# huj31415/nbody3d-webgpu

Measured on AMD Instinct MI355X. Metric: pair-interactions/s, higher is better.
Workload: dtype f32; 1 GPU; N=262144 Plummer sphere, dt=1e-3, G=1, eps2=1e-4, i-sharded over 1 GPU(s); n=262144, kernel_variant=f32pk_symw_ipl16_j1_w2048_r32t128, parallelism=1gpu

## Files before the change

### include/nbody3d_hip.h

```cpp
#ifndef NBODY3D_HIP_H
#define NBODY3D_HIP_H

#include <stddef.h>
#include <stdint.h>

#ifdef __cplusplus
extern "C" {
#endif
#if defined(__GNUC__)
#pragma GCC visibility push(default)
#endif

#define NB_ABI_VERSION 2u
#define NB_ABI_MINOR 4u

typedef struct nb_sim nb_sim;

typedef enum nb_status {
    NB_OK = 0,
    NB_ERR_INVALID = 1,
    NB_ERR_NO_DEVICE = 2,
    NB_ERR_HIP = 3,
    NB_ERR_STATE = 4,
    NB_ERR_NOMEM = 5,
    NB_ERR_COMM = 6,
    NB_NOT_READY = 7
} nb_status;

typedef enum nb_precision { NB_F32 = 0, NB_F64 = 1 } nb_precision;

#define NB_FLAG_EXT_STREAM 1u
#define NB_FLAG_LDS_ONLY 4u
#define NB_FLAG_NO_FUSE 8u
#define NB_FLAG_POISON 16u

#define NB_FLAG_JPK_FENCED 32u

#define NB_FLAG_NO_SYM 64u

#define NB_FLAG_SYM_SHARD 128u

#define NB_FLAG_WHOLE_SWEEPS 256u

#define NB_FLAG_SINGLE_SWEEPS 512u

typedef enum nb_array { NB_BODIES = 0, NB_VEL = 1, NB_ACCEL = 2, NB_JERK = 3  } nb_array;

typedef enum nb_integrator { NB_INT_LEAPFROG = 0, NB_INT_HERMITE4 = 1 } nb_integrator;

typedef struct nb_config {
    uint32_t struct_size;
    uint32_t n;
    uint32_t precision;
    uint32_t tile;
    double eps2;
    int32_t device;
    uint32_t shard_begin;
    uint32_t shard_count;
    void *ext_stream;
    void *ext_bodies;
    uint32_t force_variant;
    uint32_t jsplit;
    uint32_t flags;
    uint32_t layer_budget_mib;
    uint32_t integrator;
    uint32_t reserved[3];
} nb_config;

uint32_t nb_abi_version(void);
uint32_t nb_abi_minor(void);

int nb_device_count(void);

int nb_create(const nb_config *cfg, nb_sim **out);

void nb_destroy(nb_sim *s);

// ... 108 lines not shown
```

### nbody3d-webgpu_amd/csrc/kernels/symmetric.hip.h

```cpp
#pragma once

namespace nb {

template <typename T> struct SymRowT { T x, y, z; };
using SymRow = SymRowT<float>;

constexpr uint32_t kFlushSteps = 4096;

template <int NG>
__device__ __forceinline__ void flush_resident_sums(float (*hi)[64], const int lane, const bool flushed, nb_f2 (&ax)[NG], nb_f2 (&ay)[NG], nb_f2 (&az)[NG])
{
    if (flushed) {
#pragma unroll
        for (int c = 0; c < NG; ++c) {
            hi[6 * c + 0][lane] += ax[c].x; hi[6 * c + 1][lane] += ay[c].x; hi[6 * c + 2][lane] += az[c].x;
            hi[6 * c + 3][lane] += ax[c].y; hi[6 * c + 4][lane] += ay[c].y; hi[6 * c + 5][lane] += az[c].y;
        }
    } else {
#pragma unroll
        for (int c = 0; c < NG; ++c) {
            hi[6 * c + 0][lane] = ax[c].x; hi[6 * c + 1][lane] = ay[c].x; hi[6 * c + 2][lane] = az[c].x;
            hi[6 * c + 3][lane] = ax[c].y; hi[6 * c + 4][lane] = ay[c].y; hi[6 * c + 5][lane] = az[c].y;
        }
    }
// ... 147 lines not shown
#pragma unroll
    for (int c = 0; c < NG; ++c) {
        out[(2 * c) * 64] = SymRow{ax[c].x, ay[c].x, az[c].x};
        out[(2 * c + 1) * 64] = SymRow{ax[c].y, ay[c].y, az[c].y};
    }
}

struct SymWK { uint32_t np, nsb, W, total_hi, total_lo, n_hi, zc, ups, r_layer0, t_layer0; };
#define SYMW_PLAN_PARAMS const uint32_t W_, const uint32_t ups_, const uint32_t nsb_, const uint32_t zc_, const uint32_t r_layer0_, const uint32_t t_layer0_
typedef uint32_t nb_u4 __attribute__((ext_vector_type(4)));
template <int TAIL>
__device__ __forceinline__ void symw_record_and_tail(const uint32_t* rec_at, nb_u4& rec, uint32_t (&tail)[TAIL])
{
    static_assert(TAIL == 1 || TAIL == 4, "f32: eps2; f64: G, eps2");
    constexpr int kTailOffset = 4 * 8 + 6 * 4;
    if constexpr (TAIL == 1) {
        asm volatile("s_load_dwordx4 %0, %2, 0x0\n\ts_load_dword %1, %3, %4\n\ts_waitcnt lgkmcnt(0)"
                     : "=&s"(rec), "=&s"(tail[0]) : "s"(rec_at), "s"(__builtin_amdgcn_kernarg_segment_ptr()), "n"(kTailOffset) : "memory");
    } else {
        nb_u4 t;
        asm volatile("s_load_dwordx4 %0, %2, 0x0\n\ts_load_dwordx4 %1, %3, %4\n\ts_waitcnt lgkmcnt(0)"
                     : "=&s"(rec), "=&s"(t) : "s"(rec_at), "s"(__builtin_amdgcn_kernarg_segment_ptr()), "n"(kTailOffset) : "memory");
        tail[0] = t.x; tail[1] = t.y; tail[2] = t.z; tail[3] = t.w;
    }
}

__device__ __forceinline__ SymWK symw_plan_words(uint32_t S, uint32_t cps, uint32_t W, uint32_t ups, uint32_t nsb, uint32_t zc, uint32_t r_layer0, uint32_t t_layer0)
{
    const uint32_t H = (nsb - 1u) >> 1, n_hi = (nsb & 1u) ? 0u : nsb >> 1;
    const uint32_t total_lo = (H + 1u) * cps + zc, total_hi = total_lo + (n_hi ? cps : 0u);
    return SymWK{(nsb + (zc ? 1u : 0u)) * S, nsb, W, total_hi, total_lo, n_hi, zc, ups, r_layer0, t_layer0};
}

template <int NG, int J, bool PAIR>
__device__ __forceinline__ void symw_sweeps(const uint32_t* __restrict__ gtab, const float4* __restrict__ bodies, SymRow* __restrict__ partial, SymRow* __restrict__ spill,
                                            SYMW_PLAN_PARAMS, uint32_t* __restrict__ queue, const uint32_t npieces, const uint32_t pieces_off)
{
    static_assert(!PAIR || J == 1, "paired sweeps: one traveler per lane and sweep");
    constexpr uint32_t S = 128u * NG;
    constexpr int GW = NG < 4 ? NG : 4;
    constexpr uint32_t CH = 64u * J;
    constexpr uint32_t CPS = S / CH;
    const SymWK pl = symw_plan_words(S, CPS, W_, ups_, nsb_, zc_, r_layer0_, t_layer0_);
    const int lane = threadIdx.x & 63, wi = threadIdx.x >> 6;
    const uint32_t w = __builtin_amdgcn_readfirstlane(blockIdx.x * 4u + wi);
    const bool active = w < pl.W;
    NB_STAMP(0);
    __shared__ float red[4][6 * NG][64];
    __shared__ uint32_t fin[4];
    const uint32_t ups = pl.ups, ush = (uint32_t)__builtin_ctz(ups), ustep = 64u >> ush,
                   tab1 = 2u * (pl.np / S);
    nb_u4 rec;
    uint32_t tail[1];
    symw_record_and_tail(gtab + tab1 + 4u * (active ? w : 0u), rec, tail);
    const float eps2 = __builtin_bit_cast(float, tail[0]);
    const nb_f2 e2 = nb_f2{eps2, eps2};
    const uint32_t first_lo = pl.n_hi * pl.total_hi, first_z = first_lo + (pl.nsb - pl.n_hi) * pl.total_lo;
    const uint32_t slot = rec.w;
    NB_STAMP_LIGHT(1);
    bool first_part = true;

    auto run = [&](uint32_t u, const uint32_t uend, const uint32_t piece_layer) -> uint32_t {
        uint32_t gfin = ~0u;
        while (u < uend) {
            const uint32_t p = u >> ush;
            uint32_t g, k, total;
            if (p < first_lo) { g = p / pl.total_hi; k = p - g * pl.total_hi; total = pl.total_hi; }
            else if (p < first_z) { const uint32_t r = p - first_lo; g = pl.n_hi + r / pl.total_lo; k = r - (g - pl.n_hi) * pl.total_lo; total = pl.total_lo; }
            else { g = pl.nsb; k = p - first_z; total = pl.zc; }
            const uint32_t ring = g < pl.nsb ? total - CPS - pl.zc : 0u;
            const uint32_t both_end = g < pl.nsb ? ring + pl.zc : 0u;
            uint32_t ug_end = (p - k + total) * ups;
            if (ug_end > uend) ug_end = uend;

            nb_f2 xi[NG], yi[NG], zi[NG], mi[NG], ax[NG], ay[NG], az[NG];
            {
                const float4* rb = bodies + (size_t)g * S + lane;
#pragma unroll
                for (int c = 0; c < NG; ++c) {
                    const float4 b0 = ld4(rb + (2 * c) * 64), b1 = ld4(rb + (2 * c + 1) * 64);
                    xi[c] = nb_f2{b0.x, b1.x}; yi[c] = nb_f2{b0.y, b1.y}; zi[c] = nb_f2{b0.z, b1.z}; mi[c] = nb_f2{b0.w, b1.w};
                    ax[c] = nb_f2{0, 0}; ay[c] = nb_f2{0, 0}; az[c] = nb_f2{0, 0};
// ... 5 lines not shown
                const uint32_t q0 = u & (ups - 1u);
                bool pair = false;
                if constexpr (PAIR) pair = q0 == 0u && ug_end - u >= 2u * ups && k + 1u < both_end;
                uint32_t nun = ups - q0;
                if (nun > ug_end - u) nun = ug_end - u;
                const uint32_t s0 = q0 * ustep, s1 = s0 + nun * ustep;
                u += pair ? 2u * ups : nun;
                if (since >= kFlushSteps) {
                    flush_resident_sums<NG>(red[wi], lane, flushed, ax, ay, az);
                    flushed = true;
                    since = 0;
                }
                since += pair ? 128u : s1 - s0;
                const bool sym = k < both_end, zsweep = k >= ring && sym;
                const uint32_t d = k / CPS;
                uint32_t tb = g + 1 + d;
                if (tb >= pl.nsb) tb -= pl.nsb;
                const uint32_t tstart = k < ring ? tb * S + (k % CPS) * CH : zsweep ? pl.nsb * S + (k - ring) * CH : g * S + (k - both_end) * CH;
                const uint32_t zrow = g * pl.zc + (k - ring);
                ++k;
                if constexpr (PAIR) {
                    if (pair) {
                        const bool zsweep1 = k >= ring;
                        const uint32_t d1 = k / CPS;
                        uint32_t tb1 = g + 1 + d1;
                        if (tb1 >= pl.nsb) tb1 -= pl.nsb;
                        const uint32_t tstart1 = zsweep1 ? pl.nsb * S + (k - ring) * CH : tb1 * S + (k % CPS) * CH;
                        const uint32_t zrow1 = g * pl.zc + (k - ring);
                        ++k;
                        const float4 t0 = ld4(bodies + tstart + lane), t1 = ld4(bodies + tstart1 + lane);
                        nb_f2 tx = nb_f2{t0.x, t1.x}, ty = nb_f2{t0.y, t1.y}, tz = nb_f2{t0.z, t1.z}, tm = nb_f2{t0.w, t1.w};
                        float bx0 = 0, bx1 = 0, by0 = 0, by1 = 0, bz0 = 0, bz1 = 0;
                        if (first_part) NB_STAMP(2);
                        for (uint32_t st = 0; st < 64u; ++st) {
                            nb_f2 sx = nb_f2{0, 0}, sy = nb_f2{0, 0}, sz = nb_f2{0, 0};
#pragma unroll
                            for (int c0g = 0; c0g < NG; c0g += GW) {
#pragma unroll
                                for (int f = 0; f < 2; ++f) {
                                    nb_f2 dx[GW], dy[GW], dz[GW], d2[GW], r[GW], si[GW], sj[GW];
#pragma unroll
                                    for (int c = 0; c < GW; ++c) dx[c] = symw_sub(f, tx, xi[c0g + c]);
#pragma unroll
                                    for (int c = 0; c < GW; ++c) dy[c] = symw_sub(f, ty, yi[c0g + c]);
#pragma unroll
                                    for (int c = 0; c < GW; ++c) dz[c] = symw_sub(f, tz, zi[c0g + c]);
#pragma unroll
                                    for (int c = 0; c < GW; ++c) d2[c] = __builtin_elementwise_fma(dx[c], dx[c], e2);
#pragma unroll
                                    for (int c = 0; c < GW; ++c) d2[c] = __builtin_elementwise_fma(dy[c], dy[c], d2[c]);
#pragma unroll
                                    for (int c = 0; c < GW; ++c) d2[c] = __builtin_elementwise_fma(dz[c], dz[c], d2[c]);
#pragma unroll
                                    for (int c = 0; c < GW; ++c) r[c] = d2[c] * d2[c];
#pragma unroll
                                    for (int c = 0; c < GW; ++c) r[c] = r[c] * d2[c];
#pragma unroll
                                    for (int c = 0; c < GW; ++c) r[c] = nb_f2{nb_rsq(r[c].x), nb_rsq(r[c].y)};
#pragma unroll
                                    for (int c = 0; c < GW; ++c) si[c] = symw_mul(f, tm, r[c]);
#pragma unroll
                                    for (int c = 0; c < GW; ++c) sj[c] = mi[c0g + c] * r[c];
#pragma unroll
                                    for (int c = 0; c < GW; ++c) ax[c0g + c] = __builtin_elementwise_fma(si[c], dx[c], ax[c0g + c]);
#pragma unroll
                                    for (int c = 0; c < GW; ++c) ay[c0g + c] = __builtin_elementwise_fma(si[c], dy[c], ay[c0g + c]);
#pragma unroll
                                    for (int c = 0; c < GW; ++c) az[c0g + c] = __builtin_elementwise_fma(si[c], dz[c], az[c0g + c]);
#pragma unroll
                                    for (int c = 0; c < GW; ++c) sx = symw_fnma(f, sj[c], dx[c], sx);
#pragma unroll
                                    for (int c = 0; c < GW; ++c) sy = symw_fnma(f, sj[c], dy[c], sy);
#pragma unroll
                                    for (int c = 0; c < GW; ++c) sz = symw_fnma(f, sj[c], dz[c], sz);
                                }
                            }
                            tx = nb_f2{wave_rot1(tx.x), wave_rot1(tx.y)}; ty = nb_f2{wave_rot1(ty.x), wave_rot1(ty.y)};
                            tz = nb_f2{wave_rot1(tz.x), wave_rot1(tz.y)}; tm = nb_f2{wave_rot1(tm.x), wave_rot1(tm.y)};
                            wave_rot1_add(bx0, sx.x); wave_rot1_add(bx1, sx.y); wave_rot1_add(by0, sy.x); wave_rot1_add(by1, sy.y);
                            wave_rot1_add(bz0, sz.x); wave_rot1_add(bz1, sz.y);
                            __builtin_amdgcn_sched_barrier(0);
                        }
                        if (first_part) { NB_STAMP_LIGHT(3); first_part = false; }
                        const uint32_t home = ((uint32_t)lane + 1u) & 63u;
                        SymRow* out0 = (zsweep ? spill + (size_t)zrow * CH : partial + (size_t)(pl.t_layer0 + d) * pl.np + tstart) + home;
                        SymRow* out1 = (zsweep1 ? spill + (size_t)zrow1 * CH : partial + (size_t)(pl.t_layer0 + d1) * pl.np + tstart1) + home;
                        *out0 = SymRow{bx0, by0, bz0};
                        *out1 = SymRow{bx1, by1, bz1};
                        continue;
                    }
                }
                float tx[J], ty[J], tz[J], tm[J];
                nb_f2 bx[J], by[J], bz[J];
                const uint32_t src = ((uint32_t)lane - s0) & 63u;
#pragma unroll
                for (int uu = 0; uu < J; ++uu) {
                    const float4 t = ld4(bodies + tstart + uu * 64 + src);
                    tx[uu] = t.x; ty[uu] = t.y; tz[uu] = t.z; tm[uu] = t.w;
                    bx[uu] = nb_f2{0, 0}; by[uu] = nb_f2{0, 0}; bz[uu] = nb_f2{0, 0};
                }
                auto steps = [&](auto both) {
                    constexpr bool BOTH = decltype(both)::value;
                    for (uint32_t st = s0; st < s1; ++st) {
#pragma unroll
                        for (int uu = 0; uu < J; ++uu) {
                            const nb_f2 px = nb_f2{tx[uu], tx[uu]}, py = nb_f2{ty[uu], ty[uu]}, pz = nb_f2{tz[uu], tz[uu]}, pm = nb_f2{tm[uu], tm[uu]};
#pragma unroll
                            for (int c0g = 0; c0g < NG; c0g += GW) {
                                nb_f2 dx[GW], dy[GW], dz[GW], d2[GW], r[GW], si[GW], sj[GW];
#pragma unroll
                                for (int c = 0; c < GW; ++c) dx[c] = px - xi[c0g + c];
#pragma unroll
                                for (int c = 0; c < GW; ++c) dy[c] = py - yi[c0g + c];
#pragma unroll
// ... 112 lines not shown
            for (int j = 0; j < 4; ++j)
                if (fin[j] == gfin) { sx += red[j][3 * r + 0][lane]; sy += red[j][3 * r + 1][lane]; sz += red[j][3 * r + 2][lane]; }
            out[r * 64] = SymRow{sx, sy, sz};
        }
    }
    if (npieces) {
        for (;;) {
            uint32_t id = 0;
            if (lane == 0) id = __hip_atomic_fetch_add(queue, 1u, __ATOMIC_RELAXED, __HIP_MEMORY_SCOPE_AGENT);
            id = __builtin_amdgcn_readfirstlane(id);
            if (id >= npieces) break;
            const uint32_t pu = gtab[pieces_off + 2u * id], ll = gtab[pieces_off + 2u * id + 1u];
            (void)run(pu, pu + (ll >> 16), ll & 0xffffu);
        }
    }
    NB_STAMP(4);
}

#define SYMW_KERNEL_PARAMS const uint32_t* __restrict__ gtab, const float4* __restrict__ bodies, SymRow* __restrict__ partial, SymRow* __restrict__ spill, \
                           SYMW_PLAN_PARAMS, const float eps2_arg ,                       \
                           uint32_t* __restrict__ queue, const uint32_t npieces, const uint32_t pieces_off
#define SYMW_KERNEL_ARGS gtab, bodies, partial, spill, W_, ups_, nsb_, zc_, r_layer0_, t_layer0_, queue, npieces, pieces_off
template <int NG, int J>
__global__ __launch_bounds__(256) __attribute__((amdgpu_waves_per_eu(NG >= 4 ? 2 : 4, NG > 4 ? 2 : (NG < 4 ? 8 : 4))))
void nb_force_symw(SYMW_KERNEL_PARAMS)
{
    symw_sweeps<NG, J, false>(SYMW_KERNEL_ARGS);
}
template <int NG>
__global__ __launch_bounds__(256) __attribute__((amdgpu_waves_per_eu(2, NG > 4 ? 2 : 4)))
void nb_force_symw_pairs(SYMW_KERNEL_PARAMS)
{
    symw_sweeps<NG, 1, true>(SYMW_KERNEL_ARGS);
}

__device__ __forceinline__ double wave_rot1(double v)
{
    const long long b = __builtin_bit_cast(long long, v);
    const int lo = (int)(b & 0xffffffffll), hi = (int)(b >> 32);
    const unsigned rlo = (unsigned)__builtin_amdgcn_update_dpp(lo, lo, 0x13C, 0xF, 0xF, false);
    const unsigned rhi = (unsigned)__builtin_amdgcn_update_dpp(hi, hi, 0x13C, 0xF, 0xF, false);
    return __builtin_bit_cast(double, (long long)(((unsigned long long)rhi << 32) | rlo));
}

template <int IPL>
__global__ __launch_bounds__(256) __attribute__((amdgpu_waves_per_eu(2, 2)))
void nb_force_symw64(const uint32_t* __restrict__ gtab, const double4* __restrict__ bodies, SymRowT<double>* __restrict__ partial, SymRowT<double>* __restrict__ spill,
                     SYMW_PLAN_PARAMS, const double G_arg, const double eps2_arg ,
                     uint32_t* __restrict__ queue, const uint32_t npieces, const uint32_t pieces_off)
{
    constexpr uint32_t S = 64u * IPL, CH = 64u, CPS = S / CH;
    const SymWK pl = symw_plan_words(S, CPS, W_, ups_, nsb_, zc_, r_layer0_, t_layer0_);
    constexpr int GW = 4;
    const int lane = threadIdx.x & 63, wi = threadIdx.x >> 6;
    const uint32_t w = __builtin_amdgcn_readfirstlane(blockIdx.x * 4u + wi);
    const bool active = w < pl.W;
    __shared__ double red[4][3 * IPL][64];
    __shared__ uint32_t fin[4];
    const uint32_t ups = pl.ups, ush = (uint32_t)__builtin_ctz(ups), ustep = 64u >> ush,
                   tab1 = 2u * (pl.np / S);
    nb_u4 rec;
    uint32_t tail[4];
    symw_record_and_tail(gtab + tab1 + 4u * (active ? w : 0u), rec, tail);
    const double G = __builtin_bit_cast(double, (unsigned long long)tail[1] << 32 | tail[0]), eps2 = __builtin_bit_cast(double, (unsigned long long)tail[3] << 32 | tail[2]);
    const uint32_t first_lo = pl.n_hi * pl.total_hi, first_z = first_lo + (pl.nsb - pl.n_hi) * pl.total_lo;
    const uint32_t slot = rec.w;
// ... 586 lines not shown
```

### nbody3d-webgpu_amd/csrc/nb_engine.hip

```cpp
#include "nb_internal.h"
#include "nb_kernels.hip.h"
#include "../../include/nbody3d_hip_plan.h"

#include <hip/hip_ext.h>

#include <algorithm>
#include <cmath>
#include <cstdio>
#include <cstdlib>
#include <cstring>
#include <new>
#include <type_traits>

namespace {
thread_local std::string g_create_error = "";
}

namespace nbi {
int fail(nb_sim* s, int code, const std::string& msg)
{
    if (s) s->err = msg; else g_create_error = msg;
    return code;
}
void set_create_error(const std::string& msg) { g_create_error = msg; }
// ... 60 lines not shown
NB_PK_TABLE(pk_fused_kernel, nb_step_fused)

template <typename T>
const void* scalar_kernel(int ipl, int ls)
{
    if (ls == 1) {
        if (ipl == 1) return (const void*)&nb::nb_force<T, 1, 1>;
        if (ipl == 2) return (const void*)&nb::nb_force<T, 2, 1>;
        if (ipl == 4) return (const void*)&nb::nb_force<T, 4, 1>;
        return nullptr;
    }
    if (ipl != 1) return nullptr;
    if (ls == 4) return (const void*)&nb::nb_force<T, 1, 4>;
    if (ls == 16) return (const void*)&nb::nb_force<T, 1, 16>;
    if (ls == 64) return (const void*)&nb::nb_force<T, 1, 64>;
    return nullptr;
}

const void* sgpr_kernel(int ipl, int ws)
{
    if (ipl == 4 && ws == 5) return (const void*)&nb::nb_force_pk_sgpr<2, 4, true>;
    if (ipl == 4) return ws == 4 ? (const void*)&nb::nb_force_pk_sgpr<2, 4> : (const void*)&nb::nb_force_pk_sgpr<2, 1>;
    if (ipl == 8 && ws == 5) return (const void*)&nb::nb_force_pk_sgpr<4, 4, true>;
    if (ipl == 8) return ws == 4 ? (const void*)&nb::nb_force_pk_sgpr<4, 4> : (const void*)&nb::nb_force_pk_sgpr<4, 1>;
    return nullptr;
}

const void* rank_kernel_of(bool f64, int ipl)
{
    if (f64) return ipl == 8 ? (const void*)&nb::nb_force_symw64_rank<8> : nullptr;
    return ipl == 16 ? (const void*)&nb::nb_force_symw_rank<8> : ipl == 8 ? (const void*)&nb::nb_force_symw_rank<4> : nullptr;
}

const void* kernel_of(bool f64, const Shape& sh, bool single_sweeps = false)
{
    switch (sh.kind) {
        case kScalar: return f64 ? scalar_kernel<double>(sh.ipl, sh.ls) : scalar_kernel<float>(sh.ipl, sh.ls);
        case kPkLds: return f64 || (sh.ipl & 1) ? nullptr : pk_force_kernel(sh.ipl / 2, sh.ls, sh.x);
        case kFused: return f64 || (sh.ipl & 1) ? nullptr : pk_fused_kernel(sh.ipl / 2, sh.ls, sh.x);
        case kPkSgpr: return f64 || sh.ls != 1 || !(sh.x == 1 || sh.x == 4 || sh.x == 5) ? nullptr : sgpr_kernel(sh.ipl, sh.x);
        case kDirect:
            if (f64 || sh.ipl != 2 || sh.ls != 64) return nullptr;
            return sh.x == 1 ? (const void*)&nb::nb_step_direct<16> : sh.x == 2 ? (const void*)&nb::nb_step_direct<32> : nullptr;
        case kSym:
            if (sh.ls != 1) return nullptr;
            if (f64) return sh.ipl == 8 && sh.x == 3 ? (const void*)&nb::nb_force_symw64<8> : nullptr;
            if (sh.x == 4) return sh.ipl == 8 ? (const void*)&nb::nb_force_sym<4, 4, 2> : nullptr;
            if (sh.ipl == 4) return sh.x == 3 ? (const void*)&nb::nb_force_symw<2, 1> : nullptr;
            if (sh.ipl == 8 && sh.x == 3) return single_sweeps ? (const void*)&nb::nb_force_symw<4, 1> : (const void*)&nb::nb_force_symw_pairs<4>;
            if (sh.ipl == 16 && sh.x == 3) return single_sweeps ? (const void*)&nb::nb_force_symw<8, 1> : (const void*)&nb::nb_force_symw_pairs<8>;
            if (sh.ipl == 8) return sh.x == 1 ? (const void*)&nb::nb_force_symw<4, 2> : nullptr;
            if (sh.ipl == 16) return sh.x == 1 ? (const void*)&nb::nb_force_symw<8, 2> : nullptr;
            return nullptr;
        case kJpk:
            if (f64 || sh.ipl != 1 || sh.ls != 1) return nullptr;
            return sh.x == 4 ? (const void*)&nb::nb_step_jpk<4> : sh.x == 8 ? (const void*)&nb::nb_step_jpk<8>
                   : sh.x == 6 ? (const void*)&nb::nb_step_jpk<16> : nullptr;
        default: return nullptr;
    }
}

void plan_handle(nb_sim* s, const nb_config& cfg, int n_cu, double clock_hz, double device_mem)
{
    PlanInput in;
    if (device_mem > 0) in.device_mem = device_mem;
    in.n = s->n; in.sb = s->sb; in.sc = s->sc; in.f64 = s->f64; in.cfg = cfg; in.n_cu = n_cu; in.clock_hz = clock_hz;
    if (!s->no_device)
        in.occupancy = [f64 = s->f64](const Shape& sh, int block) {
            int occ = 0;
            const void* fn = kernel_of(f64, sh);
            if (!fn || hipOccupancyMaxActiveBlocksPerMultiprocessor(&occ, fn, block, 0) != hipSuccess) { (void)hipGetLastError(); return 0; }
            return occ;
        };
    LaunchPlan p = plan_launch(in);
    s->ipl = p.ipl; s->ls = p.ls; s->ws = p.ws; s->tl = p.tl;
    s->packed = p.packed; s->sgpr = p.sgpr; s->fused = p.fused; s->direct = p.direct; s->jpk = p.jpk; s->swap_acc = p.swap_acc;
    s->jsplit = p.jsplit; s->j_per_split = p.j_per_split; s->junits = p.junits; s->own_split0 = p.own_split0; s->own_splits = p.own_splits;
    s->sym = p.sym; s->symw = p.symw; s->sym_rank = p.sym_rank;
    s->sym_np = p.sym_np; s->sym_layers = p.sym_layers; s->sym_g0 = p.sym_g0; s->sym_g1 = p.sym_g1;
    static_assert(sizeof(s->sym_plan) == sizeof(p.sym_plan), "nb_sim::sym_plan mirrors LaunchPlan::sym_plan");
    memcpy(s->sym_plan, p.sym_plan, sizeof s->sym_plan);
    static_assert(sizeof(s->sym_rank_plan) == sizeof(p.sym_rank_plan), "nb_sim::sym_rank_plan mirrors LaunchPlan::sym_rank_plan");
    memcpy(s->sym_rank_plan, p.sym_rank_plan, sizeof s->sym_rank_plan);
// ... 62 lines not shown
        const void* b = jstream(s, s->cur);
        void* p = s->partial;
        const uint32_t* tab = s->sym_tab + ps.tab_off;
        uint32_t n = s->n, k_lo = ps.k_lo, k_hi = ps.k_hi, d0 = ps.d0;
        void* sp = s->sym_spill;
        if (s->f64) {
            double G = s->G, e2 = s->eps2;
            void* args[] = {&b, &p, &tab, &rp, &n, &G, &e2, &w0, &w1, &sp, &k_lo, &k_hi, &d0};
            launch_kernel(rank_kernel_of(true, sh.ipl), dim3(ceil_div(w1 - w0, 4u)), dim3(256), args, s->stream, t0, t1);
        } else {
            float e2 = (float)s->eps2;
            void* args[] = {&b, &p, &tab, &rp, &n, &e2, &w0, &w1, &sp, &k_lo, &k_hi, &d0};
            launch_kernel(rank_kernel_of(false, sh.ipl), dim3(ceil_div(w1 - w0, 4u)), dim3(256), args, s->stream, t0, t1);
        }
        return;
    }
    if (s->symw) {
        nb::SymWPlan pl;
        memcpy(&pl, s->sym_plan, sizeof pl);
        const void* b = jstream(s, s->cur);
        void* p = s->partial;
        const uint32_t* tab = s->sym_tab;
        void* sp = s->sym_spill;
        uint32_t* queue = s->sym_queue;
        uint32_t npieces = s->sym_pieces, pieces_off = 2u * (pl.np / ipb_of(sh)) + 4u * pl.W;
        if (npieces) (void)hipMemsetAsync(queue, 0, sizeof(uint32_t), s->stream);
        if (s->f64) {
            double G = s->G, e2 = s->eps2;
            void* args[] = {&tab, &b, &p, &sp, &pl.W, &pl.ups, &pl.nsb, &pl.zc, &pl.r_layer0, &pl.t_layer0, &G, &e2, &queue, &npieces, &pieces_off};
            launch_kernel(kernel_of(true, sh), dim3(ceil_div(pl.W, 4u)), dim3(256), args, s->stream, t0, t1);
        } else {
            float e2 = (float)s->eps2;
            void* args[] = {&tab, &b, &p, &sp, &pl.W, &pl.ups, &pl.nsb, &pl.zc, &pl.r_layer0, &pl.t_layer0, &e2, &queue, &npieces, &pieces_off};
            launch_kernel(kernel_of(false, sh, s->single_sweeps), dim3(ceil_div(pl.W, 4u)), dim3(256), args, s->stream, t0, t1);
        }
        return;
    }
    if (s->sym) {
        nb::SymPlan pl;
        memcpy(&pl, s->sym_plan, sizeof pl);
        const float4* b = (const float4*)jstream(s, s->cur);
        nb::SymRow* p = (nb::SymRow*)s->partial;
        float e2 = (float)s->eps2;
        uint32_t n = s->n;
        void* args[] = {&b, &p, &pl, &n, &e2};
        launch_kernel(kernel_of(false, sh), dim3(pl.nsb * pl.q), dim3(64 * sh.x), args, s->stream, t0, t1);
        return;
    }
    nb::SplitWindow win{0, 0xffffffffu, 0};
    uint32_t ny = s->jsplit;
    if (part == 1) { win.base = s->own_split0; ny = s->own_splits; }
    else if (part == 2) { win.hole_begin = s->own_split0; win.hole_count = s->own_splits; ny = s->jsplit - s->own_splits; }
    if (ny == 0) return;
    dim3 grid(ceil_div(s->sc, ipb_of(sh)), ny), block(nb::kBlock);
    const V4* b = (const V4*)jstream(s, s->cur);
    V4* p = (V4*)s->partial;
    T G = (T)s->G, e2 = (T)s->eps2;
    uint32_t n = s->n, sb = s->sb, sc = s->sc, jps = s->j_per_split;
    const V4* zr = (const V4*)s->zero_row;
    void* args[] = {&b, &p, &n, &sb, &sc, &G, &e2, &jps, &win, &zr};
    launch_kernel(kernel_of(s->f64, sh), grid, block, args, s->stream, t0, t1);
}

void ensure_pairs(nb_sim* s)
{
    if (!s->jpk || (s->pairs_ok && s->pairs_G == s->G)) return;
    const float4* b = (const float4*)s->bodies[s->cur];
// ... 428 lines not shown
        s->hermite = true;
        fj_shape(s->n, s->f64, n_cu, &s->fj_chunks, &s->fj_per);
        s->jsplit = s->fj_chunks; s->j_per_split = s->fj_per;
        s->variant = std::string("hermite4_") + (s->f64 ? "f64" : "f32pk") + "_c" + std::to_string(s->fj_chunks) + "_j" + std::to_string(s->fj_per);
        const size_t hrow = 4 * s->esz;
        NB_HIPC(hipMalloc(&s->bodies[0], hrow * s->n));
        s->own_bodies = true;
        for (void** p : {&s->vel, &s->acc, &s->jerk, &s->hx, &s->hv}) NB_HIPC(hipMalloc(p, hrow * s->n));
        NB_HIPC(hipMalloc(&s->fj_part, (size_t)2 * hrow * s->fj_chunks * s->n));
        NB_HIPC(hipMalloc(&s->zero_row, 64));
        NB_HIPC(hipMemsetAsync(s->zero_row, 0, 64, s->stream));
        s->diag_chunk = nb::kTile * std::min(16u, std::max(1u, s->n / 16384u));
        s->diag_blocks = ceil_div(s->sc, nb::kDiagRows) * ceil_div(s->n, s->diag_chunk);
        NB_HIPC(hipMalloc((void**)&s->diag, sizeof(double) * 5 * s->diag_blocks));
        *out = s;
        return NB_OK;
    }
    plan_handle(s, cfg, n_cu, clock_hz, (double)prop.totalGlobalMem);
    if (s->sym && (!s->sym_rank || s->sym_local) && !cfg.force_variant) {
        size_t free_b = 0, total_b = 0;
        auto need = [&]() { return 3.0 * s->esz * (double)sym_layer_rows(s) * s->sym_layers + 12.0 * s->esz * s->sym_np; };
        if (hipMemGetInfo(&free_b, &total_b) == hipSuccess && need() > 0.9 * (double)free_b) {
            nb_config fit = cfg;
            fit.layer_budget_mib = (uint32_t)std::max(1.0, 0.6 * (double)free_b / 1048576.0);
            plan_handle(s, fit, n_cu, clock_hz, (double)prop.totalGlobalMem);
            if (s->sym && need() > 0.9 * (double)free_b) {
                cfg.flags |= NB_FLAG_NO_SYM;
                plan_handle(s, cfg, n_cu, clock_hz, (double)prop.totalGlobalMem);
            }
        }
    }
    if (!kernel_of(s->f64, shape_of(s))) return bail(NB_ERR_INVALID, "nb_create: no kernel for shape " + s->variant);
    s->single_sweeps = (cfg.flags & NB_FLAG_SINGLE_SWEEPS) != 0;

    const size_t row = 4 * s->esz;
    if (cfg.ext_bodies) { s->bodies[0] = cfg.ext_bodies; s->own_bodies = false; }
    else {
        const size_t rows = s->sym ? s->sym_np : s->n;
        NB_HIPC(hipMalloc(&s->bodies[0], row * rows));
        if (s->sym) NB_HIPC(hipMemset(s->bodies[0], 0, row * rows));
        s->own_bodies = true;
        if (s->fused) NB_HIPC(hipMalloc(&s->bodies[1], row * s->n));
    }
    NB_HIPC(hipMalloc(&s->vel, row * s->sc));
    NB_HIPC(hipMalloc(&s->acc, row * s->sc));
    auto alloc_partial = [&](size_t bytes) -> hipError_t {
        if (s->partial) return hipErrorInvalidValue;
        s->partial_bytes = bytes;
        return hipMalloc(&s->partial, bytes);
    };
    if (s->sym) {
        NB_HIPC(alloc_partial((size_t)3 * s->esz * sym_layer_rows(s) * s->sym_layers));
        if (s->sym_rank) NB_HIPC(hipMalloc(&s->sym_A, 4 * s->esz * s->sym_np));
        if (s->sym_spill_rows) {
            NB_HIPC(hipMalloc(&s->sym_spill, (size_t)3 * s->esz * s->sym_spill_rows));
            NB_HIPC(hipMemset(s->sym_spill, 0, (size_t)3 * s->esz * s->sym_spill_rows));
        }
        if (s->symw && s->sym_pieces) {
            NB_HIPC(hipMalloc((void**)&s->sym_queue, 64));
            NB_HIPC(hipMemset(s->sym_queue, 0, 64));
        }
        if (s->symw) {
            NB_HIPC(hipMalloc((void**)&s->sym_tab, sizeof(uint32_t) * s->sym_tab_host.size()));
            NB_HIPC(hipMemcpy(s->sym_tab, s->sym_tab_host.data(), sizeof(uint32_t) * s->sym_tab_host.size(), hipMemcpyHostToDevice));
        }
    } else if (!s->fused) {
// ... 744 lines not shown
```

### nbody3d-webgpu_amd/csrc/nb_internal.h

```cpp
#pragma once
#include "../../include/nbody3d_hip.h"
#include "nb_plan.h"

#include <hip/hip_runtime.h>

#include <cstdint>
#include <string>
#include <vector>

struct nb_events { hipEvent_t e[8]; bool two, xchg, rs; };

struct nb_rccl;

struct nb_frame_slot {
    float* h_bodies = nullptr;
    float* h_speed = nullptr;
    float* d_bodies = nullptr;
    float* d_speed = nullptr;
    hipEvent_t packed = nullptr;
    hipEvent_t landed = nullptr;
    uint64_t step = 0;
    bool in_flight = false, valid = false;
};

// ... 21 lines not shown
    uint32_t diag_blocks = 0, diag_chunk = 256;
    double dt = 0.0, G = 0.0;
    bool params_set = false, uploaded = false;
    uint64_t steps_done = 0;
    int ipl = 1, ls = 1;
    bool packed = false;
    bool sgpr = false;
    int ws = 1;
    int tl = 1;
    bool fused = false;
    bool direct = false;
    bool jpk = false;
    void* pairs[2] = {nullptr, nullptr};
    bool pairs_ok = false;
    double pairs_G = 0.0;
    void* jpartial = nullptr;
    uint32_t* tickets = nullptr;
    uint32_t junits = 0;
    bool poison = false;
    bool jpk_fenced = false;
    int acc_parity = 0;
    bool swap_acc = false;
    uint32_t jsplit = 1, j_per_split = 0;
    bool sym = false;
    uint32_t sym_np = 0, sym_layers = 0;
    uint32_t sym_plan[16] = {0};
    bool symw = false;
    uint32_t* sym_tab = nullptr;
    std::vector<uint32_t> sym_tab_host;
    void* sym_spill = nullptr;
    uint32_t sym_spill_rows = 0;
    uint32_t sym_pieces = 0;
    bool single_sweeps = false;
    uint32_t* sym_queue = nullptr;
    bool sym_rank = false;
    uint32_t sym_g0 = 0, sym_g1 = 0;
    uint32_t sym_rank_plan[16] = {0};
    std::vector<nbp::LaunchPlan::SymPass> sym_passes;
    uint32_t sym_pass = 0;
    bool sym_local = false;
    void* sym_A = nullptr;
    std::string variant, err;
    nb_exchange_fn xfn = nullptr;
    nb_exchange_wait_fn xwait = nullptr;
    void* xuser = nullptr;
    bool gather_pending = false;
    uint32_t own_split0 = 0, own_splits = 0;
    nb_rccl* rccl = nullptr;
    bool timing = false;
    struct graph_slot {
        hipGraph_t graph = nullptr;
        hipGraphExec_t exec = nullptr;
        double dt = 0.0, G = 0.0;
        int parity = 0;
    } graphs[2];
    bool graphs_ok = true;
    std::vector<nb_events> pool;
    std::vector<nb_events> pending;
    size_t pool_next = 0;
    hipStream_t frame_stream = nullptr;
    static constexpr int kFrameSlots = 4;
    nb_frame_slot frame[kFrameSlots];
    int frame_next = 0;
    int frame_latest = -1;
    int n_cu = 256;
    struct field_buf { void* p = nullptr; size_t cap = 0; } fld_pts, fld_acc, fld_phi, fld_part;
// ... 27 lines not shown
```

### nbody3d-webgpu_amd/nbody3d_amd/capi.py

```python
import ctypes as C
import os

import numpy as np

_PKG = os.path.dirname(os.path.abspath(__file__))
_LIB_PATH = os.environ.get("NB_ENGINE_LIB") or os.path.normpath(os.path.join(_PKG, "..", "csrc", "libnbody3d_hip.so"))

NB_F32, NB_F64 = 0, 1
NB_FLAG_EXT_STREAM = 1
NB_FLAG_LDS_ONLY = 4
NB_FLAG_NO_FUSE = 8
NB_FLAG_POISON = 16
NB_FLAG_JPK_FENCED = 32
NB_FLAG_NO_SYM = 64
NB_FLAG_SYM_SHARD = 128
NB_FLAG_WHOLE_SWEEPS = 256
NB_FLAG_SINGLE_SWEEPS = 512
NB_RCCL_ID_BYTES = 128
NB_RCCL_OVERLAP = 1
NB_MULTI_PEER, NB_MULTI_RCCL, NB_MULTI_PEER_OVERLAP = 0, 1, 2
NB_NOT_READY = 7
NB_FIELD_AT_BODIES, NB_FIELD_F64, NB_FIELD_DEVICE = 1, 2, 4
NB_INT_LEAPFROG, NB_INT_HERMITE4 = 0, 1
INTEGRATORS = {"leapfrog": NB_INT_LEAPFROG, "hermite4": NB_INT_HERMITE4}
STATUS = {0: "NB_OK", 1: "NB_ERR_INVALID", 2: "NB_ERR_NO_DEVICE", 3: "NB_ERR_HIP",
          4: "NB_ERR_STATE", 5: "NB_ERR_NOMEM", 6: "NB_ERR_COMM", 7: "NB_NOT_READY"}
ABI_VERSION = 2
ABI_MINOR = 3


class NBodyError(RuntimeError):
    def __init__(self, code, msg):
        super().__init__("%s: %s" % (STATUS.get(code, code), msg))
        self.code = code


class nb_config(C.Structure):
    _fields_ = [
        ("struct_size", C.c_uint32), ("n", C.c_uint32), ("precision", C.c_uint32), ("tile", C.c_uint32),
        ("eps2", C.c_double), ("device", C.c_int32), ("shard_begin", C.c_uint32), ("shard_count", C.c_uint32),
        ("ext_stream", C.c_void_p), ("ext_bodies", C.c_void_p),
        ("force_variant", C.c_uint32), ("jsplit", C.c_uint32), ("flags", C.c_uint32), ("layer_budget_mib", C.c_uint32),
        ("integrator", C.c_uint32), ("reserved", C.c_uint32 * 3),
    ]


class nb_plan_info(C.Structure):
    _fields_ = [("struct_size", C.c_uint32)] + [(k, C.c_uint32) for k in (
        "kind", "ipl", "ls", "x", "jsplit", "j_per_split", "own_split0", "own_splits",
        "sym", "symw", "sym_rank", "sym_np", "sym_layers", "sym_g0", "sym_g1")] + [
# ... 619 lines not shown
```

Before: 6896 billion pair-interactions/s.

## Stage paired-sweep travelers in LDS instead of rotating them across lanes

For the 16-resident paired symmetric kernel, each lane writes its traveler body into a per-wave LDS ring once. Every sweep step then reads the neighbour's traveler by address rotation, replacing the eight cross-lane rotations per step. The loop is unrolled by two with double-buffered traveler registers so the LDS read can overlap the pair math. The trade is extra LDS traffic and 8 KiB of shared memory per workgroup, with the old rotation path kept behind a new flag.

```diff
diff --git a/include/nbody3d_hip.h b/include/nbody3d_hip.h
--- a/include/nbody3d_hip.h
+++ b/include/nbody3d_hip.h
@@ -43,6 +43,8 @@
 #define NB_FLAG_WHOLE_SWEEPS 256u
 
 #define NB_FLAG_SINGLE_SWEEPS 512u
+
+#define NB_FLAG_ROTATE_TRAVELERS 1024u
 
 typedef enum nb_array { NB_BODIES = 0, NB_VEL = 1, NB_ACCEL = 2, NB_JERK = 3  } nb_array;
 
diff --git a/nbody3d-webgpu_amd/csrc/kernels/symmetric.hip.h b/nbody3d-webgpu_amd/csrc/kernels/symmetric.hip.h
--- a/nbody3d-webgpu_amd/csrc/kernels/symmetric.hip.h
+++ b/nbody3d-webgpu_amd/csrc/kernels/symmetric.hip.h
@@ -203,11 +203,42 @@
     return SymWK{(nsb + (zc ? 1u : 0u)) * S, nsb, W, total_hi, total_lo, n_hi, zc, ups, r_layer0, t_layer0};
 }
 
-template <int NG, int J, bool PAIR>
+__device__ __forceinline__ uint32_t symw_traveler_slots()
+{
+    __shared__ __attribute__((aligned(1024))) nb_v4f trav[4][2][64];
+    return (uint32_t)(uintptr_t)&trav[0][0][0];
+}
+
+#define SYMW_PAIR_TERMS(tx, ty, tz, tm, sx, sy, sz)                                                                              \
+    _Pragma("unroll") for (int c0g = 0; c0g < NG; c0g += GW) {                                                                   \
+        _Pragma("unroll") for (int f = 0; f < 2; ++f) {                                                                          \
+            nb_f2 dx[GW], dy[GW], dz[GW], d2[GW], r[GW], si[GW], sj[GW];                                                         \
+            _Pragma("unroll") for (int c = 0; c < GW; ++c) dx[c] = symw_sub(f, tx, xi[c0g + c]);                       \
+            _Pragma("unroll") for (int c = 0; c < GW; ++c) dy[c] = symw_sub(f, ty, yi[c0g + c]);                                 \
+            _Pragma("unroll") for (int c = 0; c < GW; ++c) dz[c] = symw_sub(f, tz, zi[c0g + c]);                                 \
+            _Pragma("unroll") for (int c = 0; c < GW; ++c) d2[c] = __builtin_elementwise_fma(dx[c], dx[c], e2);        \
+            _Pragma("unroll") for (int c = 0; c < GW; ++c) d2[c] = __builtin_elementwise_fma(dy[c], dy[c], d2[c]);               \
+            _Pragma("unroll") for (int c = 0; c < GW; ++c) d2[c] = __builtin_elementwise_fma(dz[c], dz[c], d2[c]);               \
+            _Pragma("unroll") for (int c = 0; c < GW; ++c) r[c] = d2[c] * d2[c];                                       \
+            _Pragma("unroll") for (int c = 0; c < GW; ++c) r[c] = r[c] * d2[c];                                                  \
+            _Pragma("unroll") for (int c = 0; c < GW; ++c) r[c] = nb_f2{nb_rsq(r[c].x), nb_rsq(r[c].y)};                         \
+            _Pragma("unroll") for (int c = 0; c < GW; ++c) si[c] = symw_mul(f, tm, r[c]);  \
+            _Pragma("unroll") for (int c = 0; c < GW; ++c) sj[c] = mi[c0g + c] * r[c];           \
+            _Pragma("unroll") for (int c = 0; c < GW; ++c) ax[c0g + c] = __builtin_elementwise_fma(si[c], dx[c], ax[c0g + c]);   \
+            _Pragma("unroll") for (int c = 0; c < GW; ++c) ay[c0g + c] = __builtin_elementwise_fma(si[c], dy[c], ay[c0g + c]);   \
+            _Pragma("unroll") for (int c = 0; c < GW; ++c) az[c0g + c] = __builtin_elementwise_fma(si[c], dz[c], az[c0g + c]);   \
+            _Pragma("unroll") for (int c = 0; c < GW; ++c) sx = symw_fnma(f, sj[c], dx[c], sx);                                  \
+            _Pragma("unroll") for (int c = 0; c < GW; ++c) sy = symw_fnma(f, sj[c], dy[c], sy);                                  \
+            _Pragma("unroll") for (int c = 0; c < GW; ++c) sz = symw_fnma(f, sj[c], dz[c], sz);                                  \
+        }                                                                                                                        \
+    }
+
+template <int NG, int J, bool PAIR, bool TRAV_LDS = false>
 __device__ __forceinline__ void symw_sweeps(const uint32_t* __restrict__ gtab, const float4* __restrict__ bodies, SymRow* __restrict__ partial, SymRow* __restrict__ spill,
                                             SYMW_PLAN_PARAMS, uint32_t* __restrict__ queue, const uint32_t npieces, const uint32_t pieces_off)
 {
     static_assert(!PAIR || J == 1, "paired sweeps: one traveler per lane and sweep");
+    static_assert(!TRAV_LDS || (PAIR && NG == 8), "travelers in LDS: the paired sweeps of the 16-resident kernel (with 8 residents four workgroups share a CU's LDS)");
     constexpr uint32_t S = 128u * NG;
     constexpr int GW = NG < 4 ? NG : 4;
     constexpr uint32_t CH = 64u * J;
@@ -219,6 +250,8 @@
     NB_STAMP(0);
     __shared__ float red[4][6 * NG][64];
     __shared__ uint32_t fin[4];
+    uint32_t trav_home = 0;
+    if constexpr (TRAV_LDS) trav_home = symw_traveler_slots() + (uint32_t)wi * 2048u + (uint32_t)lane * 16u;
     const uint32_t ups = pl.ups, ush = (uint32_t)__builtin_ctz(ups), ustep = 64u >> ush,
                    tab1 = 2u * (pl.np / S);
     nb_u4 rec;
@@ -290,54 +323,44 @@
                         nb_f2 tx = nb_f2{t0.x, t1.x}, ty = nb_f2{t0.y, t1.y}, tz = nb_f2{t0.z, t1.z}, tm = nb_f2{t0.w, t1.w};
                         float bx0 = 0, bx1 = 0, by0 = 0, by1 = 0, bz0 = 0, bz1 = 0;
                         if (first_part) NB_STAMP(2);
-                        for (uint32_t st = 0; st < 64u; ++st) {
-                            nb_f2 sx = nb_f2{0, 0}, sy = nb_f2{0, 0}, sz = nb_f2{0, 0};
-#pragma unroll
-                            for (int c0g = 0; c0g < NG; c0g += GW) {
-#pragma unroll
-                                for (int f = 0; f < 2; ++f) {
-                                    nb_f2 dx[GW], dy[GW], dz[GW], d2[GW], r[GW], si[GW], sj[GW];
-#pragma unroll
-                                    for (int c = 0; c < GW; ++c) dx[c] = symw_sub(f, tx, xi[c0g + c]);
-#pragma unroll
-                                    for (int c = 0; c < GW; ++c) dy[c] = symw_sub(f, ty, yi[c0g + c]);
-#pragma unroll
-                                    for (int c = 0; c < GW; ++c) dz[c] = symw_sub(f, tz, zi[c0g + c]);
-#pragma unroll
-                                    for (int c = 0; c < GW; ++c) d2[c] = __builtin_elementwise_fma(dx[c], dx[c], e2);
-#pragma unroll
-                                    for (int c = 0; c < GW; ++c) d2[c] = __builtin_elementwise_fma(dy[c], dy[c], d2[c]);
-#pragma unroll
-                                    for (int c = 0; c < GW; ++c) d2[c] = __builtin_elementwise_fma(dz[c], dz[c], d2[c]);
-#pragma unroll
-                                    for (int c = 0; c < GW; ++c) r[c] = d2[c] * d2[c];
-#pragma unroll
-                                    for (int c = 0; c < GW; ++c) r[c] = r[c] * d2[c];
-#pragma unroll
-                                    for (int c = 0; c < GW; ++c) r[c] = nb_f2{nb_rsq(r[c].x), nb_rsq(r[c].y)};
-#pragma unroll
-                                    for (int c = 0; c < GW; ++c) si[c] = symw_mul(f, tm, r[c]);
-#pragma unroll
-                                    for (int c = 0; c < GW; ++c) sj[c] = mi[c0g + c] * r[c];
-#pragma unroll
-                                    for (int c = 0; c < GW; ++c) ax[c0g + c] = __builtin_elementwise_fma(si[c], dx[c], ax[c0g + c]);
-#pragma unroll
-                                    for (int c = 0; c < GW; ++c) ay[c0g + c] = __builtin_elementwise_fma(si[c], dy[c], ay[c0g + c]);
-#pragma unroll
-                                    for (int c = 0; c < GW; ++c) az[c0g + c] = __builtin_elementwise_fma(si[c], dz[c], az[c0g + c]);
-#pragma unroll
-                                    for (int c = 0; c < GW; ++c) sx = symw_fnma(f, sj[c], dx[c], sx);
-#pragma unroll
-                                    for (int c = 0; c < GW; ++c) sy = symw_fnma(f, sj[c], dy[c], sy);
-#pragma unroll
-                                    for (int c = 0; c < GW; ++c) sz = symw_fnma(f, sj[c], dz[c], sz);
-                                }
+                        if constexpr (TRAV_LDS) {
+                            typedef __attribute__((address_space(3))) nb_v4f lds_v4f;
+                            uint32_t at = trav_home;
+                            *(lds_v4f*)(uintptr_t)at = nb_v4f{t0.x, t1.x, t0.y, t1.y};
+                            *(lds_v4f*)(uintptr_t)(at + 1024u) = nb_v4f{t0.z, t1.z, t0.w, t1.w};
+                            auto request = [&](nb_f2& x, nb_f2& y, nb_f2& z, nb_f2& m) {
+                                at = (at & ~0x3f0u) | ((at - 16u) & 0x3f0u);
+                                const nb_v4f xy = *(const lds_v4f*)(uintptr_t)at, zm = *(const lds_v4f*)(uintptr_t)(at + 1024u);
+                                x = nb_f2{xy.x, xy.y}; y = nb_f2{xy.z, xy.w}; z = nb_f2{zm.x, zm.y}; m = nb_f2{zm.z, zm.w};
+                                __builtin_amdgcn_sched_barrier(0);
+                            };
+                            auto sums_move_on = [&](const nb_f2 sx, const nb_f2 sy, const nb_f2 sz) {
+                                wave_rot1_add(bx0, sx.x); wave_rot1_add(bx1, sx.y); wave_rot1_add(by0, sy.x); wave_rot1_add(by1, sy.y);
+                                wave_rot1_add(bz0, sz.x); wave_rot1_add(bz1, sz.y);
+                                __builtin_amdgcn_sched_barrier(0);
+                            };
+                            __builtin_amdgcn_s_waitcnt(0xc07f);
+                            nb_f2 ux, uy, uz, um;
+                            for (uint32_t st = 0; st < 64u; st += 2u) {
+                                nb_f2 sx = nb_f2{0, 0}, sy = nb_f2{0, 0}, sz = nb_f2{0, 0};
+                                request(ux, uy, uz, um);
+                                SYMW_PAIR_TERMS(tx, ty, tz, tm, sx, sy, sz)
+                                sums_move_on(sx, sy, sz);
+                                sx = nb_f2{0, 0}; sy = nb_f2{0, 0}; sz = nb_f2{0, 0};
+                                request(tx, ty, tz, tm);
+                                SYMW_PAIR_TERMS(ux, uy, uz, um, sx, sy, sz)
+                                sums_move_on(sx, sy, sz);
                             }
-                            tx = nb_f2{wave_rot1(tx.x), wave_rot1(tx.y)}; ty = nb_f2{wave_rot1(ty.x), wave_rot1(ty.y)};
-                            tz = nb_f2{wave_rot1(tz.x), wave_rot1(tz.y)}; tm = nb_f2{wave_rot1(tm.x), wave_rot1(tm.y)};
-                            wave_rot1_add(bx0, sx.x); wave_rot1_add(bx1, sx.y); wave_rot1_add(by0, sy.x); wave_rot1_add(by1, sy.y);
-                            wave_rot1_add(bz0, sz.x); wave_rot1_add(bz1, sz.y);
-                            __builtin_amdgcn_sched_barrier(0);
+                        } else {
+                            for (uint32_t st = 0; st < 64u; ++st) {
+                                nb_f2 sx = nb_f2{0, 0}, sy = nb_f2{0, 0}, sz = nb_f2{0, 0};
+                                SYMW_PAIR_TERMS(tx, ty, tz, tm, sx, sy, sz)
+                                tx = nb_f2{wave_rot1(tx.x), wave_rot1(tx.y)}; ty = nb_f2{wave_rot1(ty.x), wave_rot1(ty.y)};
+                                tz = nb_f2{wave_rot1(tz.x), wave_rot1(tz.y)}; tm = nb_f2{wave_rot1(tm.x), wave_rot1(tm.y)};
+                                wave_rot1_add(bx0, sx.x); wave_rot1_add(bx1, sx.y); wave_rot1_add(by0, sy.x); wave_rot1_add(by1, sy.y);
+                                wave_rot1_add(bz0, sz.x); wave_rot1_add(bz1, sz.y);
+                                __builtin_amdgcn_sched_barrier(0);
+                            }
                         }
                         if (first_part) { NB_STAMP_LIGHT(3); first_part = false; }
                         const uint32_t home = ((uint32_t)lane + 1u) & 63u;
@@ -516,6 +539,12 @@
 void nb_force_symw_pairs(SYMW_KERNEL_PARAMS)
 {
     symw_sweeps<NG, 1, true>(SYMW_KERNEL_ARGS);
+}
+template <int NG>
+__global__ __launch_bounds__(256) __attribute__((amdgpu_waves_per_eu(2, 2)))
+void nb_force_symw_pairs_lds(SYMW_KERNEL_PARAMS)
+{
+    symw_sweeps<NG, 1, true, true>(SYMW_KERNEL_ARGS);
 }
 
 __device__ __forceinline__ double wave_rot1(double v)
diff --git a/nbody3d-webgpu_amd/csrc/nb_engine.hip b/nbody3d-webgpu_amd/csrc/nb_engine.hip
--- a/nbody3d-webgpu_amd/csrc/nb_engine.hip
+++ b/nbody3d-webgpu_amd/csrc/nb_engine.hip
@@ -116,7 +116,7 @@
     return ipl == 16 ? (const void*)&nb::nb_force_symw_rank<8> : ipl == 8 ? (const void*)&nb::nb_force_symw_rank<4> : nullptr;
 }
 
-const void* kernel_of(bool f64, const Shape& sh, bool single_sweeps = false)
+const void* kernel_of(bool f64, const Shape& sh, bool single_sweeps = false, bool rotate_travelers = false)
 {
     switch (sh.kind) {
         case kScalar: return f64 ? scalar_kernel<double>(sh.ipl, sh.ls) : scalar_kernel<float>(sh.ipl, sh.ls);
@@ -132,7 +132,8 @@
             if (sh.x == 4) return sh.ipl == 8 ? (const void*)&nb::nb_force_sym<4, 4, 2> : nullptr;
             if (sh.ipl == 4) return sh.x == 3 ? (const void*)&nb::nb_force_symw<2, 1> : nullptr;
             if (sh.ipl == 8 && sh.x == 3) return single_sweeps ? (const void*)&nb::nb_force_symw<4, 1> : (const void*)&nb::nb_force_symw_pairs<4>;
-            if (sh.ipl == 16 && sh.x == 3) return single_sweeps ? (const void*)&nb::nb_force_symw<8, 1> : (const void*)&nb::nb_force_symw_pairs<8>;
+            if (sh.ipl == 16 && sh.x == 3)
+                return single_sweeps ? (const void*)&nb::nb_force_symw<8, 1> : rotate_travelers ? (const void*)&nb::nb_force_symw_pairs<8> : (const void*)&nb::nb_force_symw_pairs_lds<8>;
             if (sh.ipl == 8) return sh.x == 1 ? (const void*)&nb::nb_force_symw<4, 2> : nullptr;
             if (sh.ipl == 16) return sh.x == 1 ? (const void*)&nb::nb_force_symw<8, 2> : nullptr;
             return nullptr;
@@ -261,7 +262,7 @@
         } else {
             float e2 = (float)s->eps2;
             void* args[] = {&tab, &b, &p, &sp, &pl.W, &pl.ups, &pl.nsb, &pl.zc, &pl.r_layer0, &pl.t_layer0, &e2, &queue, &npieces, &pieces_off};
-            launch_kernel(kernel_of(false, sh, s->single_sweeps), dim3(ceil_div(pl.W, 4u)), dim3(256), args, s->stream, t0, t1);
+            launch_kernel(kernel_of(false, sh, s->single_sweeps, s->rotate_travelers), dim3(ceil_div(pl.W, 4u)), dim3(256), args, s->stream, t0, t1);
         }
         return;
     }
@@ -756,6 +757,7 @@
     }
     if (!kernel_of(s->f64, shape_of(s))) return bail(NB_ERR_INVALID, "nb_create: no kernel for shape " + s->variant);
     s->single_sweeps = (cfg.flags & NB_FLAG_SINGLE_SWEEPS) != 0;
+    s->rotate_travelers = (cfg.flags & NB_FLAG_ROTATE_TRAVELERS) != 0;
 
     const size_t row = 4 * s->esz;
     if (cfg.ext_bodies) { s->bodies[0] = cfg.ext_bodies; s->own_bodies = false; }
diff --git a/nbody3d-webgpu_amd/csrc/nb_internal.h b/nbody3d-webgpu_amd/csrc/nb_internal.h
--- a/nbody3d-webgpu_amd/csrc/nb_internal.h
+++ b/nbody3d-webgpu_amd/csrc/nb_internal.h
@@ -77,6 +77,7 @@
     uint32_t sym_spill_rows = 0;
     uint32_t sym_pieces = 0;
     bool single_sweeps = false;
+    bool rotate_travelers = false;
     uint32_t* sym_queue = nullptr;
     bool sym_rank = false;
     uint32_t sym_g0 = 0, sym_g1 = 0;
diff --git a/nbody3d-webgpu_amd/nbody3d_amd/capi.py b/nbody3d-webgpu_amd/nbody3d_amd/capi.py
--- a/nbody3d-webgpu_amd/nbody3d_amd/capi.py
+++ b/nbody3d-webgpu_amd/nbody3d_amd/capi.py
@@ -16,6 +16,7 @@
 NB_FLAG_SYM_SHARD = 128
 NB_FLAG_WHOLE_SWEEPS = 256
 NB_FLAG_SINGLE_SWEEPS = 512
+NB_FLAG_ROTATE_TRAVELERS = 1024
 NB_RCCL_ID_BYTES = 128
 NB_RCCL_OVERLAP = 1
 NB_MULTI_PEER, NB_MULTI_RCCL, NB_MULTI_PEER_OVERLAP = 0, 1, 2
```

Measured after the change: 6949 billion pair-interactions/s (median of 6 runs). About the same (+0.8%).
